# IC3Net/IC3Net

Hardware: AMD Instinct MI355X
Metric: env-steps/sec (agents x envs x steps), rollout hot path (higher is better)
Workload: dtype f32

## Files before the change

ic3net_amd/csrc/bptt_kernels.hip:

```cpp
#include <hip/hip_runtime.h>

#include <algorithm>
#include <cstddef>
#include <type_traits>
#include <vector>

#include "enc_bwd.hpp"
#include "ic3_common.hpp"
#include "ps_common.hpp"

extern "C" int ic3_lstm_gates_backward_given(const float* gates, float* xh, int ldx, const float* h_prev, const void* lstm_wp3_bwd,
                                             const float* c_prev, const float* dh, const float* dc, float* dgates, float* dc_prev,
                                             float* dbias_partials, int accumulate, float* dxh, const float* row_live,
                                             const float* row_keep, const float* dhead, const float* w_heads, int OT, int R, int H,
                                             ic3_stream stream);

namespace ic3 {

typedef float bp_f32x2 __attribute__((ext_vector_type(2)));
typedef float bp_f32x4 __attribute__((ext_vector_type(4)));
typedef float bp_f32x16 __attribute__((ext_vector_type(16)));

__device__ __forceinline__ __amdgpu_buffer_rsrc_t bp_rsrc(const void* base, long long bytes)
{
    const uint32_t n = bytes <= 0 ? 0u : (bytes > 0xffffffffll ? 0xffffffffu : (uint32_t)bytes);
    return __builtin_amdgcn_make_buffer_rsrc(const_cast<void*>(base), 0, n, 0x00020000);
}
__device__ __forceinline__ float bp_load1(__amdgpu_buffer_rsrc_t r, int voff, int soff = 0)
{
    return __builtin_bit_cast(float, __builtin_amdgcn_raw_buffer_load_b32(r, voff, soff, 0));
}
__device__ __forceinline__ bp_f32x4 bp_load4(__amdgpu_buffer_rsrc_t r, int voff, int soff = 0)
{
    return __builtin_bit_cast(bp_f32x4, __builtin_amdgcn_raw_buffer_load_b128(r, voff, soff, 0));
}
__device__ __forceinline__ void bp_store4(bp_f32x4 v, __amdgpu_buffer_rsrc_t r, int voff, int soff = 0)
{
    __builtin_amdgcn_raw_buffer_store_b128(__builtin_bit_cast(ps_u32x4, v), r, voff, soff, 0);
}
__device__ __forceinline__ void bp_mfma(bp_f32x16& acc, float x, float y)
{
    acc = __builtin_amdgcn_mfma_f32_32x32x2f32(x, y, acc, 0, 0, 0);
}
template <int N>
__device__ __forceinline__ void bp_zero(bp_f32x16* acc)
{
#pragma unroll
    for (int n = 0; n < N; ++n)
#pragma unroll
        for (int i = 0; i < 16; ++i) acc[n][i] = 0.0f;
}

struct KSlice {
    long long q0, nq;
    int nstages;
};
__device__ __forceinline__ KSlice bp_kslice(long long Q, int rows_per_wg, int KT)
{
    const long long q0 = (long long)blockIdx.x * rows_per_wg;
    long long nq = Q - q0;
    if (nq > rows_per_wg) nq = rows_per_wg;
    if (nq < 0) nq = 0;
    return KSlice{ q0, nq, (int)((nq + KT - 1) / KT) };
}

struct CommBwdArgs {
    const float* dxh;
    const float* h_prev;
    const int32_t* alive;
    const int32_t* gate;
    const float* cw;
    const float* out_scale;
    float* dh_out;
    float* dcw_part;
    int ldd, E, N, ept, tiles, mode_avg, accumulate;
};

template <int H>
__global__ __launch_bounds__(2 * H, (H <= 128) ? 3 : 1) void comm_bwd_kernel(const CommBwdArgs a)
{
    constexpr int NT = 2 * H, H4 = H / 4, LDA = H + 4, LDA4 = LDA / 4, MB = H / 32, PER = 64 * H4 / NT;
    IC3_DYNAMIC_LDS(float, smem);
    float* const Am = smem;
    bp_f32x4* const Am4 = reinterpret_cast<bp_f32x4*>(smem);
    float* const sg = smem + 64 * LDA;
    float* const sal = sg + 64;
    const int tid = threadIdx.x, lane = tid & 63, w = tid >> 6, li = lane & 31, lh = lane >> 5;
    const int col = 32 * w + li;
    const int N = a.N;
    bp_f32x16 acc2[MB];
    bp_zero<MB>(acc2);
    const __amdgpu_buffer_rsrc_t rcw = bp_rsrc(a.cw, (long long)H * H * 4);

    for (int tile = blockIdx.x; tile < a.tiles; tile += gridDim.x) {
        const int e0 = tile * a.ept;
        const int ne = (a.E - e0) < a.ept ? (a.E - e0) : a.ept;
        const int rows = ne * N;
        const long long r0 = (long long)e0 * N;
        const __amdgpu_buffer_rsrc_t rdi = bp_rsrc(a.dxh + r0 * a.ldd, ((long long)(rows - 1) * a.ldd + H) * 4);
        const __amdgpu_buffer_rsrc_t rdd = bp_rsrc(a.dxh + r0 * a.ldd + H, ((long long)(rows - 1) * a.ldd + H) * 4);
        const __amdgpu_buffer_rsrc_t rhp = bp_rsrc(a.h_prev + r0 * H, (long long)rows * H * 4);
        bp_f32x4 v[PER];
#pragma unroll
        for (int i = 0; i < PER; ++i) {
            const int idx = tid + i * NT, row = idx / H4, c4 = idx - row * H4;
            v[i] = bp_load4(rdi, (row * a.ldd + 4 * c4) * 4);
        }
        float mg = 0.f, mal = 0.f;
        if (tid < 64 && tid < rows) {
            mal = a.alive ? (float)a.alive[r0 + tid] : 1.0f;
            mg = mal * (a.gate ? (float)a.gate[r0 + tid] : 1.0f);
        }
        bp_f32x16 acc1[2];
#pragma unroll
        for (int rt = 0; rt < 2; ++rt)
#pragma unroll
            for (int reg = 0; reg < 16; ++reg)
                acc1[rt][reg] = bp_load1(rdd, (4 * lh * a.ldd + col) * 4, (32 * rt + (reg & 3) + 8 * (reg >> 2)) * a.ldd * 4);
#pragma unroll
        for (int i = 0; i < PER; ++i) Am4[(tid + i * NT) / H4 * LDA4 + (tid + i * NT) % H4] = v[i];
        if (tid < 64) {
            sg[tid] = mg;
            sal[tid] = mal;
        }
        float hpv[32];
#pragma unroll
        for (int s = 0; s < 32; ++s) hpv[s] = bp_load1(rhp, (lh * H + col) * 4, 2 * s * H * 4);
        __syncthreads();
        for (int item = tid; item < ne * H4; item += NT) {
            const int el = item / H4, c4 = item - el * H4;
            float na = 0.f;
            for (int j = 0; j < N; ++j) na += sal[el * N + j];
            const int n_alive = (int)na;
            const float scale = (a.mode_avg && n_alive > 1) ? 1.0f / (float)(n_alive - 1) : 1.0f;
            bp_f32x4 S = { 0.f, 0.f, 0.f, 0.f };
            for (int i = 0; i < N; ++i) S = mask_fma4(sg[el * N + i], Am4[(el * N + i) * LDA4 + c4], S);
            for (int j = 0; j < N; ++j) {
                const float m = sg[el * N + j];
                const bp_f32x4 x = Am4[(el * N + j) * LDA4 + c4];
                Am4[(el * N + j) * LDA4 + c4] = comm_out4(m, S, x, scale);
            }
        }
        __syncthreads();
        float wv[4], wn[4];
#pragma unroll
        for (int j = 0; j < 4; ++j) wv[j] = bp_load1(rcw, (4 * lh * H + col) * 4, j * H * 4);
#pragma unroll 2
        for (int kb = 0; kb < H / 8; ++kb) {
#pragma unroll
            for (int j = 0; j < 4; ++j) wn[j] = bp_load1(rcw, (4 * lh * H + col) * 4, (8 * (kb + 1) + j) * H * 4);
            const bp_f32x4 a0 = Am4[li * LDA4 + 2 * kb + lh];
            const bp_f32x4 a1 = Am4[(32 + li) * LDA4 + 2 * kb + lh];
#pragma unroll
            for (int j = 0; j < 4; ++j) {
                bp_mfma(acc1[0], a0[j], wv[j]);
                bp_mfma(acc1[1], a1[j], wv[j]);
            }
#pragma unroll
            for (int j = 0; j < 4; ++j) wv[j] = wn[j];
        }
        {
            const __amdgpu_buffer_rsrc_t rout = bp_rsrc(a.dh_out + r0 * H, (long long)rows * H * 4);
            const __amdgpu_buffer_rsrc_t rsc = bp_rsrc(a.out_scale ? a.out_scale + r0 : a.dh_out, a.out_scale ? (long long)rows * 4 : 0);
#pragma unroll
            for (int rt = 0; rt < 2; ++rt)
#pragma unroll
                for (int reg = 0; reg < 16; ++reg) {
                    const int lc = 32 * rt + (reg & 3) + 8 * (reg >> 2);
                    float o = acc1[rt][reg];
                    if (a.out_scale) o *= bp_load1(rsc, 4 * lh * 4, lc * 4);
                    __builtin_amdgcn_raw_buffer_store_b32(__builtin_bit_cast(int, o), rout, (4 * lh * H + col) * 4, lc * H * 4, 0);
                }
        }
#pragma unroll 4
        for (int s = 0; s < 32; ++s) {
#pragma unroll
            for (int mb = 0; mb < MB; ++mb) bp_mfma(acc2[mb], Am[(2 * s + lh) * LDA + 32 * mb + li], hpv[s]);
        }
        __syncthreads();
    }
    float* dst = a.dcw_part + (size_t)blockIdx.x * H * H;
#pragma unroll
    for (int mb = 0; mb < MB; ++mb)
#pragma unroll
        for (int reg = 0; reg < 16; ++reg) {
            const int k = 32 * mb + (reg & 3) + 8 * (reg >> 2) + 4 * lh;
            if (a.accumulate) dst[k * H + col] += acc2[mb][reg];
            else dst[k * H + col] = acc2[mb][reg];
        }
}

__global__ __launch_bounds__(256) void dh_copy_kernel(const float* __restrict__ dxh, int ldd, const float* __restrict__ out_scale,
                                                      float* __restrict__ dh_out, long long R, int H4)
{
    for (long long i = (long long)blockIdx.x * blockDim.x + threadIdx.x; i < R * H4; i += (long long)gridDim.x * blockDim.x) {
        const long long row = i / H4;
        const int c4 = (int)(i - row * H4);
        bp_f32x4 v = *reinterpret_cast<const bp_f32x4*>(dxh + row * ldd + 4 * H4 + 4 * c4);
        if (out_scale) v *= out_scale[row];
        reinterpret_cast<bp_f32x4*>(dh_out)[i] = v;
    }
}

struct WGradArgs {
    const float* inp;
    const float* h;
    const float* dg;
    const float* row_live;
    float* part;
    long long Q;
    int ldi, rows_per_wg;
};

template <int H>
__global__ __launch_bounds__(256, 2) void lstm_wgrad_kernel(const WGradArgs a)
{
    constexpr bool WIDE = H == 256;
    constexpr int HT = WIDE ? 128 : H;
    constexpr int KT = 16, XW = 2 * HT, DW = 128, MB = HT / 32, NB = 2, NT = 256;
    constexpr int X4R = XW / 4, D4R = DW / 4;
    constexpr int XPT = KT * X4R / NT, DPT = KT * D4R / NT;
    static_assert(XPT >= 1 && DPT == 2 && (NT % X4R) == 0, "staging split");
    IC3_DYNAMIC_LDS(float, smem);
    constexpr int SW = KT * (XW + DW);
    const int tid = threadIdx.x, lane = tid & 63, w = tid >> 6, li = lane & 31, lh = lane >> 5;
    const int wm = w & 1, wn = w >> 1;
    const int ny = blockIdx.y;
    const KSlice sl = bp_kslice(a.Q, a.rows_per_wg, KT);
    const long long q0 = sl.q0, nq = sl.nq;
    const int nstages = sl.nstages;
    const __amdgpu_buffer_rsrc_t ri = bp_rsrc(a.inp + q0 * a.ldi, nq > 0 ? ((nq - 1) * a.ldi + H) * 4 : 0);
    const __amdgpu_buffer_rsrc_t rh = bp_rsrc(a.h + q0 * H, nq * H * 4);
    const __amdgpu_buffer_rsrc_t rd = bp_rsrc(a.dg + q0 * 4 * H + ny * DW, nq > 0 ? ((nq - 1) * 4 * H + DW) * 4 : 0);
    const __amdgpu_buffer_rsrc_t rl = bp_rsrc(a.row_live ? a.row_live + q0 : a.h, a.row_live ? nq * 4 : 0);
    const int xrow = tid / X4R, xc4 = tid - xrow * X4R;
    const bool x_is_h = WIDE ? blockIdx.z != 0 : xc4 >= H / 4;
    const int xvoff = x_is_h ? (xrow * H + 4 * xc4 - (WIDE ? 0 : H)) * 4 : (xrow * a.ldi + 4 * xc4) * 4;
    const int xstep = (NT / X4R) * (x_is_h ? H : a.ldi) * 4;
    const int drow = tid / D4R, dc4 = tid - drow * D4R;
    const int dvoff = (drow * 4 * H + 4 * dc4) * 4;

    bp_f32x4 xr[XPT], dr[DPT];
    auto fetch = [&](int s) {
        const int qb = s * KT;
#pragma unroll
        for (int i = 0; i < XPT; ++i) {
            if (x_is_h) {
                xr[i] = bp_load4(rh, xvoff + i * xstep, qb * H * 4);
                if (a.row_live) xr[i] *= bp_load1(rl, (xrow + i * (NT / X4R)) * 4, qb * 4);
            } else {
                xr[i] = bp_load4(ri, xvoff + i * xstep, qb * a.ldi * 4);
            }
        }
#pragma unroll
        for (int i = 0; i < DPT; ++i) dr[i] = bp_load4(rd, dvoff + i * (NT / D4R) * 4 * H * 4, qb * 4 * H * 4);
    };
    auto stash = [&](int b) {
        bp_f32x4* X4 = reinterpret_cast<bp_f32x4*>(smem + b * SW);
        bp_f32x4* D4 = reinterpret_cast<bp_f32x4*>(smem + b * SW + KT * XW);
#pragma unroll
        for (int i = 0; i < XPT; ++i) X4[tid + i * NT] = xr[i];
#pragma unroll
        for (int i = 0; i < DPT; ++i) D4[tid + i * NT] = dr[i];
    };
    bp_f32x16 acc[MB][NB];
    bp_zero<MB * NB>(&acc[0][0]);
    if (nstages > 0) {
        fetch(0);
        stash(0);
    }
    __syncthreads();
    for (int s = 0; s < nstages; ++s) {
// ... 88 lines not shown
        for (int j = 0; j < 8; ++j) dv[j] = bp_load1(rd, doff, (qb + j) * 4 * H * 4);
    };
    auto stash = [&](int b) {
        ps_u32x4* f = frag + b * SQ;
        ps_u32x4 pl[3];
#pragma unroll
        for (int i = 0; i < NGX; ++i) {
            const int g = tid + i * NT, c = g % XW, kg = g / XW;
            ps_split_frag(ps_f32x4{ xv[i][0], xv[i][1], xv[i][2], xv[i][3] }, ps_f32x4{ xv[i][4], xv[i][5], xv[i][6], xv[i][7] }, pl);
#pragma unroll
            for (int p = 0; p < 3; ++p) f[(p * 2 + kg) * XW + c] = pl[p];
        }
        ps_split_frag(ps_f32x4{ dv[0], dv[1], dv[2], dv[3] }, ps_f32x4{ dv[4], dv[5], dv[6], dv[7] }, pl);
#pragma unroll
        for (int p = 0; p < 3; ++p) f[3 * 2 * XW + (p * 2 + dkg) * DW + dcol] = pl[p];
    };
    bp_f32x16 acc[MB][NB];
    bp_zero<MB * NB>(&acc[0][0]);
    fetch(0);
    stash(0);
    fetch(1);
    __syncthreads();
#pragma unroll 1
    for (int s = 0; s < nstages; ++s) {
        const ps_u32x4* fx = frag + (s & 1) * SQ;
        const ps_u32x4* fd = fx + 3 * 2 * XW;
        ps_u32x4 bf[3][NB];
#pragma unroll
        for (int p = 0; p < 3; ++p)
#pragma unroll
            for (int nb = 0; nb < NB; ++nb) bf[p][nb] = fd[(p * 2 + lh) * DW + 64 * wn + 32 * nb + li];
        stash((s + 1) & 1);
#pragma unroll
        for (int mb = 0; mb < MB; ++mb) {
            ps_u32x4 af[3];
#pragma unroll
            for (int p = 0; p < 3; ++p) af[p] = fx[(p * 2 + lh) * XW + wm * HT + 32 * mb + li];
#pragma unroll
            for (int pb = 0; pb < 3; ++pb)
#pragma unroll
                for (int nb = 0; nb < NB; ++nb)
#pragma unroll
                    for (int pa = 2; pa >= 0; --pa)
                        acc[mb][nb] = __builtin_amdgcn_mfma_f32_32x32x16_bf16(__builtin_bit_cast(wg_bf16x8, af[pa]),
                                                                              __builtin_bit_cast(wg_bf16x8, bf[pb][nb]), acc[mb][nb], 0, 0, 0);
        }
        fetch(s + 2);
        __syncthreads();
    }
    float* dst = a.part + (size_t)blockIdx.x * 2 * H * 4 * H;
    const int m0 = WIDE ? (int)blockIdx.z * XW : 0;
#pragma unroll
    for (int mb = 0; mb < MB; ++mb)
#pragma unroll
        for (int nb = 0; nb < NB; ++nb)
#pragma unroll
            for (int reg = 0; reg < 16; ++reg) {
                const int m = m0 + wm * HT + 32 * mb + (reg & 3) + 8 * (reg >> 2) + 4 * lh;
                dst[(size_t)m * 4 * H + DW * ny + 64 * wn + 32 * nb + li] = acc[mb][nb][reg];
            }
}

__global__ __launch_bounds__(256) void wgrad_reduce_kernel(const float* __restrict__ part, int nparts, int n, float* __restrict__ dW,
                                                           int accumulate)
{
    const int i = blockIdx.x * blockDim.x + threadIdx.x;
    if (i >= n) return;
    float s = 0.f;
    for (int p = 0; p < nparts; ++p) s += part[(size_t)p * n + i];
    dW[i] = accumulate ? dW[i] + s : s;
}

}

extern "C" int ic3_comm_backward_partials(int E, int N)
{
    if (E <= 0 || N <= 0 || N > 64) return 0;
    const int ept = 64 / N, tiles = (E + ept - 1) / ept;
    constexpr int cap = 512;
    const int rounds = (tiles + cap - 1) / cap;
    return (tiles + rounds - 1) / rounds;
}

extern "C" int ic3_comm_backward(const float* dxh, int ldd, const float* h_prev, const int32_t* alive, const int32_t* gate,
                                 const float* c_weight, const float* out_scale, float* dh_out,
                                 float* dcw_partials, int accumulate, int E, int N, int H, int mode_avg, int comm_zero,
                                 ic3_stream stream)
{
    using namespace ic3;
    if (!dxh || !dh_out || E <= 0 || N <= 0) return fail(-22, "ic3_comm_backward: null argument");
    if (ldd < 2 * H || (ldd & 3) || (H & 3)) return fail(-22, "ic3_comm_backward: ldd a multiple of 4, >= 2 * hid_size");
    hipStream_t s = (hipStream_t)stream;
    if (comm_zero) {
        const long long R = (long long)E * N, n4 = R * (H / 4);
        const int blocks = (int)std::min<long long>((n4 + 255) / 256, 4096);
        return launch_kernel(dh_copy_kernel, dim3(blocks), dim3(256), 0, s, dxh, ldd, out_scale, dh_out, R, H / 4);
    }
    if (!h_prev || !c_weight || !dcw_partials) return fail(-22, "ic3_comm_backward: null argument");
    if (H != 64 && H != 128 && H != 256) return fail(-38, "ic3_comm_backward: hid_size 64 / 128 / 256");
    if (N > 64) return fail(-38, "ic3_comm_backward: at most 64 agents per env");
    const int ept = 64 / N, tiles = (E + ept - 1) / ept;
    if ((long long)64 * ldd * 4 >= (1ll << 31)) return fail(-22, "ic3_comm_backward: row stride too large");
    const CommBwdArgs a{ dxh, h_prev, alive, gate, c_weight, out_scale, dh_out, dcw_partials, ldd, E, N, ept, tiles,
                         mode_avg, accumulate };
    const int grid = ic3_comm_backward_partials(E, N);
    const size_t lds = ((size_t)64 * (H + 4) + 128) * sizeof(float);
    const auto kernel = H == 256 ? comm_bwd_kernel<256> : H == 128 ? comm_bwd_kernel<128> : comm_bwd_kernel<64>;
    const int rc = launch_kernel(kernel, dim3(grid), dim3(2 * H), lds, s, a);
    return rc < 0 ? rc : grid;
}

struct WGradPlan {
    int ks;
    long long per;
    bool fits;
};
static WGradPlan wgrad_plan(long long Q, int ny, long long row_floats)
{
    int ks = 2 * ic3::device_cus() / ny;
    const long long most = (Q + 15) / 16;
    if (ks > most) ks = (int)most;
    if (ks < 1) ks = 1;
    const long long per = ((Q + ks - 1) / ks + 15) / 16 * 16;
    return WGradPlan{ ks, per, per * row_floats * 4 < (1ll << 31) };
}

static int wgrad_reduce(const float* scratch, int ks, int n, float* dW, int accumulate, hipStream_t s)
{
    const int rc = ic3::launch_kernel(ic3::wgrad_reduce_kernel, dim3((n + 255) / 256), dim3(256), 0, s, scratch, ks, n, dW, accumulate);
    return rc < 0 ? rc : ks;
}

static WGradPlan wgrad_plan_rounds(long long Q, int ny, long long row_floats)
{
    WGradPlan pl = wgrad_plan(Q, ny, row_floats);
    const long long most = (Q + 15) / 16;
    const int round = pl.ks;
    for (long long m = 2; !pl.fits && round * m <= most; ++m) {
        pl.ks = (int)(round * m);
        pl.per = ((Q + pl.ks - 1) / pl.ks + 15) / 16 * 16;
        pl.fits = pl.per * row_floats * 4 < (1ll << 31);
    }
    return pl;
}
static WGradPlan lstm_wgrad_plan(long long Q, int H, long long row_floats)
{
    return H == 256 ? wgrad_plan_rounds(Q, 16, row_floats) : wgrad_plan(Q, 4 * H / 128, row_floats);
}
static WGradPlan rnn_wgrad_plan(long long Q, int H, long long row_floats)
{
    return H == 256 ? wgrad_plan_rounds(Q, 4, row_floats) : wgrad_plan(Q, 1, row_floats);
}

static int lstm_weight_grad(const float* inp, int ldi, const float* h_prev, const float* dgates, const float* row_live, long long Q,
                            int H, float* dW, int accumulate, int split, float* scratch, ic3_stream stream)
{
    using namespace ic3;
    if (!inp || !h_prev || !dgates || !dW || !scratch || Q <= 0) return fail(-22, "ic3_lstm_weight_grad: null argument");
    if (ldi < H || (ldi & 3)) return fail(-22, "ic3_lstm_weight_grad: ldi a multiple of 4, >= hid_size");
    const WGradPlan pl = lstm_wgrad_plan(Q, H, std::max(ldi, 4 * H));
    if (!pl.fits) return fail(-22, "ic3_lstm_weight_grad: a K slice must stay below 2 GB per operand (32-bit buffer offsets)");
    const WGradArgs a{ inp, h_prev, dgates, row_live, scratch, Q, ldi, (int)pl.per };
    hipStream_t s = (hipStream_t)stream;
    const auto kernel = split ? (H == 256 ? lstm_wgrad_split_kernel<256> : H == 128 ? lstm_wgrad_split_kernel<128> : lstm_wgrad_split_kernel<64>)
                              : (H == 256 ? lstm_wgrad_kernel<256> : H == 128 ? lstm_wgrad_kernel<128> : lstm_wgrad_kernel<64>);
    const int HT = H == 256 ? 128 : H;
    const size_t lds = split ? (size_t)2 * 3 * 2 * (2 * HT + 128) * 16 : (size_t)2 * 16 * (2 * HT + 128) * sizeof(float);
    const dim3 grid = H == 256 ? dim3(pl.ks, 8, 2) : dim3(pl.ks, 4 * H / 128);
    if (const int rc = launch_kernel(kernel, grid, dim3(256), lds, s, a); rc < 0) return rc;
    return wgrad_reduce(scratch, pl.ks, 2 * H * 4 * H, dW, accumulate, s);
}

extern "C" size_t ic3_lstm_weight_grad_scratch_floats(long long Q, int H)
{
    if (Q <= 0 || (H != 64 && H != 128)) return 0;
    return (size_t)wgrad_plan(Q, 4 * H / 128, 0).ks * 2 * H * 4 * H;
}

extern "C" int ic3_lstm_weight_grad(const float* inp, int ldi, const float* h_prev, const float* dgates, const float* row_live,
                                    long long Q, int H, float* dW, int accumulate, int split, float* scratch, ic3_stream stream)
{
    if (H != 64 && H != 128) return ic3::fail(-38, "ic3_lstm_weight_grad: hid_size 64 / 128");
    return lstm_weight_grad(inp, ldi, h_prev, dgates, row_live, Q, H, dW, accumulate, split, scratch, stream);
}

extern "C" size_t ic3_lstm_weight_grad_wide_scratch_floats(long long Q, int H, int ldi)
{
    if (Q <= 0 || (H != 64 && H != 128 && H != 256)) return 0;
    return (size_t)lstm_wgrad_plan(Q, H, std::max(ldi, 4 * H)).ks * 2 * H * 4 * H;
}

extern "C" int ic3_lstm_weight_grad_wide(const float* inp, int ldi, const float* h_prev, const float* dgates, const float* row_live,
// ... 16 lines not shown
        const ic3_tj_cfg& c = env->tj;
        const int WW = env->dims.window * env->dims.window, hdr = c.vocab_type ? 4 : 2;
        pl = enc_bwd_plan(c.E, c.N, c.N, H, env->dims.grid_h * env->dims.grid_w, hdr + WW);
    }
    return pl.csplit ? 1 : 0;
}

namespace ic3 {
struct BpttSide {
    hipStream_t stream = nullptr;
    hipEvent_t fork = nullptr, join = nullptr;
    bool ready = false;
};
static BpttSide* bptt_side()
{
    static BpttSide side[65];
    int dev = 0;
    if (hipGetDevice(&dev) != hipSuccess || dev < -1 || dev >= 64) return nullptr;
    BpttSide& sd = side[dev + 1];
    if (!sd.ready) {
        if (!sd.stream && hipStreamCreateWithFlags(&sd.stream, hipStreamNonBlocking) != hipSuccess) return nullptr;
        if ((!sd.fork && hipEventCreateWithFlags(&sd.fork, hipEventDisableTiming) != hipSuccess) ||
            (!sd.join && hipEventCreateWithFlags(&sd.join, hipEventDisableTiming) != hipSuccess))
            return nullptr;
        sd.ready = true;
    }
    return &sd;
}

template <class B>
static int window_open(const char* fn, const char* sname, const ic3_env* env, const B* b, int (*supported)(const ic3_env*, int),
                       const char* needs, bool ot_enosys)
{
    const std::string f = std::string(fn) + ": ";
    if (!env || !b) return fail(-22, f + "null argument");
    if (b->struct_size != sizeof(B))
        return fail(-22, f + sname + " has " + std::to_string(b->struct_size) + " bytes, this library's has " +
                             std::to_string(sizeof(B)) + " (header / library version mismatch)");
    if (b->T <= 0 || b->E <= 0 || b->N <= 0 || b->E != env->dims.E || b->N != env->dims.N)
        return fail(-22, f + "T, E, N must be positive and E, N the handle's");
    if (!supported(env, b->H)) return fail(-38, f + needs);
    if (ot_enosys) {
        if (b->OT < 1) return fail(-22, f + "OT >= 1");
        if (b->OT > 16) return fail(-38, f + "at most 16 output columns");
    } else if (b->OT < 1 || b->OT > 16) {
        return fail(-22, f + "1 <= OT <= 16");
    }
    return 0;
}

static int encoder_tail(ic3_env* env, const int32_t* snaps, int64_t snap_words, int T, const float* g, int ldg, int64_t g_step,
                        int H, float* work, int enc_first, bool window, ic3_stream stream)
{
    if (window) return ic3_env_encode_backward_window(env, snaps, snap_words, T, g, ldg, g_step, H, work, enc_first, stream);
    for (int t = T - 1; t >= 0; --t) {
        const int rc = ic3_env_encode_backward_accumulate(env, snaps + (size_t)t * snap_words, g + (size_t)t * g_step, ldg, H, work,
                                                          enc_first, stream);
        if (rc < 0) return rc;
        enc_first = 0;
    }
    return 0;
}

struct BpttCell {
    float* gates;
    const float* c_prev;
    const float* h_prev;
    float* dh;
    float* dc;
    bool cut;
    float* dxh;
    float* dbias;
    const float* row_live;
    const float* row_keep;
    const float* dhead;
    const float* w_heads;
    int OT;
    const void* lstm_wp3_bwd;
    const int32_t* alive;
    const int32_t* gate;
    const float* c_weight;
    const float* out_scale;
    float* dcw;
    hipEvent_t ev0, ev1;
};
static int bptt_cell_backward(const char* fn, const BpttCell& q, int Ec, int N, int H, int mode_avg, int comm_zero, hipStream_t sc)
{
    ic3_stream scv = (ic3_stream)sc;
    if (q.ev0 && hipEventRecord(q.ev0, sc) != hipSuccess) return fail(-5, std::string(fn) + ": hipEventRecord of a gate event failed");
    int rc = ic3_lstm_gates_backward_given(q.gates, nullptr, 0, nullptr, q.lstm_wp3_bwd, q.c_prev, q.cut ? nullptr : q.dh,
                                           q.cut ? nullptr : q.dc, q.gates, q.dc, q.dbias, 1, q.dxh, q.row_live, q.row_keep, q.dhead,
                                           q.dhead ? q.w_heads : nullptr, q.OT, Ec * N, H, scv);
    if (rc < 0) return rc;
    if (q.ev1 && hipEventRecord(q.ev1, sc) != hipSuccess) return fail(-5, std::string(fn) + ": hipEventRecord of a gate event failed");
    return ic3_comm_backward(q.dxh, 2 * H, q.h_prev, q.alive, q.gate, q.c_weight, q.out_scale, q.dh, q.dcw, 1, Ec, N, H, mode_avg,
                             comm_zero, scv);
}
}

static int bptt_passes_backward(ic3_env* env, const ic3_bptt_passes* b, ic3_stream stream)
{
    using namespace ic3;
    if (const int rc = window_open("ic3_bptt_backward (ic3_bptt_passes)", "ic3_bptt_passes", env, b, ic3_bptt_backward_supported,
                                   "hid_size 64 / 128 / 256, <= 64 agents, a grid whose encoder backward runs in its partial-sums form",
                                   false);
        rc < 0)
        return rc;
    const int T = b->T, E = b->E, N = b->N, H = b->H, P = b->passes;
    if (P < 2) return fail(-22, "ic3_bptt_backward (ic3_bptt_passes): passes >= 2 (one pass: ic3_bptt_backward)");
    if (ic3_env_encode_backward_window_work(env, H) <= 0)
        return fail(-38, "ic3_bptt_backward (ic3_bptt_passes): needs a configuration with ic3_env_encode_backward_window (the ring form)");
    if (!b->gates || !b->hs || !b->cs || !b->dhead || !b->snaps || !b->lstm_wp3_bwd || !b->w_heads || !b->dh || !b->dc || !b->dxh ||
        !b->dbias_partials || !b->enc_work || b->t_first < 0)
        return fail(-22, "ic3_bptt_backward (ic3_bptt_passes): null argument");
    if (!b->comm_zero && (!b->c_weight || !b->dcw_partials)) return fail(-22, "ic3_bptt_backward (ic3_bptt_passes): the passes' C.weight and partials");
    const long long R = (long long)E * N;
    if (b->dxh_step < R * 2 * H) return fail(-22, "ic3_bptt_backward (ic3_bptt_passes): dxh_step >= E * N * 2 * hid_size (the ring form)");
    for (int i = 0; i < P; ++i) {
        if (!b->gates[i] || !b->hs[i] || !b->cs[i] || !b->dxh[i] || !b->dbias_partials[i] ||
            (!b->comm_zero && (!b->c_weight[i] || !b->dcw_partials[i])))
            return fail(-22, "ic3_bptt_backward (ic3_bptt_passes): null argument of pass " + std::to_string(i));
    }
    if (R * 4 * H * 4 >= (1ll << 32))
        return fail(-22, "ic3_bptt_backward (ic3_bptt_passes): rows * 4 * hid_size floats must stay below 4 GB (the gate launch's 32-bit buffer "
                         "offsets)");
    if (b->detach_gap > 0 && (b->row_keep || b->keep_before))
        return fail(-22, "ic3_bptt_backward (ic3_bptt_passes): detach_gap > 0 with row_keep / keep_before (a detached step has no dc for "
                         "row_keep to scale: lock-step windows carry detach_gap, collection-mode windows the row factors)");
    hipStream_t s = (hipStream_t)stream;
    for (int t = T - 1; t >= 0; --t) {
        const bool detached = b->detach_gap > 0 && (b->t_first + t + 1) % b->detach_gap == 0;
        const float* keep_here = b->row_keep ? b->row_keep + (size_t)t * R : nullptr;
        const float* keep_front = t > 0 ? (b->row_keep ? b->row_keep + (size_t)(t - 1) * R : nullptr) : b->keep_before;
        for (int i = P - 1; i >= 0; --i) {
            const bool last = i == P - 1;
            BpttCell q{};
            q.gates = b->gates[i] + (size_t)t * R * 4 * H;
            q.c_prev = b->cs[i] + (size_t)t * R * H;
            q.h_prev = b->hs[i] + (size_t)t * R * H;
            q.dh = b->dh;
            q.dc = b->dc;
            q.cut = detached && last;
            q.dxh = b->dxh[i] + (size_t)t * (size_t)b->dxh_step;
            q.dbias = b->dbias_partials[i];
            q.dhead = last ? b->dhead + (size_t)t * R * b->OT : nullptr;
            q.w_heads = b->w_heads;
            q.OT = b->OT;
            q.lstm_wp3_bwd = b->lstm_wp3_bwd;
            q.alive = (b->alive && b->alive[t]) ? b->alive[t] : nullptr;
            q.gate = (b->gate && b->gate[t]) ? b->gate[t] : nullptr;
            q.c_weight = b->comm_zero ? nullptr : b->c_weight[i];
            q.dcw = b->comm_zero ? nullptr : b->dcw_partials[i];
            q.row_keep = last ? keep_here : nullptr;
            q.out_scale = i == 0 ? keep_front : nullptr;
            if (const int rc = bptt_cell_backward("ic3_bptt_backward (ic3_bptt_passes)", q, E, N, H, b->mode_avg, b->comm_zero, s); rc < 0) return rc;
        }
    }
    for (int i = 0; i < P; ++i) {
        const int rc = ic3_env_encode_backward_window(env, b->snaps, b->snap_words, T, b->dxh[i], 2 * H, b->dxh_step, H, b->enc_work,
                                                      (i == 0 && b->enc_first) ? 1 : 0, stream);
        if (rc < 0) return rc;
    }
    return 0;
}

static int bptt_walk_backward(ic3_env* env, const ic3_bptt_walk* b, ic3_stream stream)
{
    using namespace ic3;
    const char* const fn = "ic3_bptt_backward (ic3_bptt_walk)";
    const std::string f = std::string(fn) + ": ";
    if (const int rc = window_open(fn, "ic3_bptt_walk", env, b, ic3_bptt_backward_supported,
                                   "hid_size 64 / 128 / 256, <= 64 agents, a grid whose encoder backward runs in its partial-sums form",
                                   false);
        rc < 0)
        return rc;
    if (!b->gates || !b->hs || !b->cs || !b->dhead || !b->snaps || !b->lstm_wp3_bwd || !b->w_heads || !b->dh || !b->dc || !b->dxh ||
        !b->dbias_partials || !b->enc_work)
        return fail(-22, f + "null argument");
    const long long R = (long long)b->E * b->N;
    if (b->dxh_step < R * 2 * b->H || ic3_env_encode_backward_window_work(env, b->H) <= 0)
        return fail(-22, f + "dxh_step >= E * N * 2 * hid_size, on a configuration with ic3_env_encode_backward_window (the walk needs "
                             "the ring)");
    if (b->detach_gap > 0 && b->row_keep)
        return fail(-22, f + "detach_gap > 0 with row_keep (a detached step has no dc for row_keep to scale: lock-step windows carry "
                             "detach_gap, collection-mode windows row_live / row_keep)");
    if (R >= (1ll << 31) || b->max_workgroups < 0) return fail(-22, f + "R < 2^31, max_workgroups >= 0");
    if (const int rc = lstm_gates_backward_walk(b, stream); rc < 0) return rc;
    return ic3_env_encode_backward_window(env, b->snaps, b->snap_words, b->T, b->dxh, 2 * b->H, b->dxh_step, b->H, b->enc_work,
                                          b->enc_first, stream);
}

extern "C" int ic3_bptt_first_chain_envs(int E, int N)
{
    if (E < 128 || N <= 0) return E;
    return (E / 2) & ~63;
}

extern "C" int ic3_bptt_backward(ic3_env* env, const ic3_bptt* b, ic3_stream stream)
{
    using namespace ic3;
    static_assert(offsetof(ic3_bptt_passes, magic) == offsetof(ic3_bptt, T), "the tag sits where ic3_bptt holds T");
    if (b && (uint32_t)b->T == IC3_BPTT_PASSES_MAGIC)
        return bptt_passes_backward(env, reinterpret_cast<const ic3_bptt_passes*>(b), stream);
    static_assert(offsetof(ic3_bptt_walk, magic) == offsetof(ic3_bptt, T), "the tag sits where ic3_bptt holds T");
    static_assert(sizeof(ic3_bptt_walk) != sizeof(ic3_bptt) && sizeof(ic3_bptt_walk) != sizeof(ic3_bptt_passes),
                  "the descriptors are told apart by their sizes too");
    if (b && (uint32_t)b->T == IC3_BPTT_WALK_MAGIC) return bptt_walk_backward(env, reinterpret_cast<const ic3_bptt_walk*>(b), stream);
    if (const int rc = window_open("ic3_bptt_backward", "ic3_bptt", env, b, ic3_bptt_backward_supported,
                                   "hid_size 64 / 128 / 256, <= 64 agents, a grid whose encoder backward runs in its partial-sums form",
                                   false);
        rc < 0)
        return rc;
    const int T = b->T, E = b->E, N = b->N, H = b->H;
    if (!b->gates || !b->hs || !b->cs || !b->dhead || !b->snaps || !b->lstm_wp3_bwd || !b->w_heads || !b->dh || !b->dc || !b->dxh ||
        !b->dbias_partials || !b->enc_work)
        return fail(-22, "ic3_bptt_backward: null argument");
    if (!b->comm_zero && (!b->c_weight || !b->dcw_partials)) return fail(-22, "ic3_bptt_backward: C.weight and its partials");
    if (b->dxh_step && (b->dxh_step < (long long)E * N * 2 * H || ic3_env_encode_backward_window_work(env, H) <= 0))
        return fail(-22, "ic3_bptt_backward: dxh_step >= E * N * 2 * hid_size, on a configuration with ic3_env_encode_backward_window");
    if (b->detach_gap > 0 && b->row_keep)
        return fail(-22, "ic3_bptt_backward: detach_gap > 0 with row_keep (a detached step has no dc for row_keep to scale: lock-step "
                         "windows carry detach_gap, collection-mode windows row_live / row_keep)");
    const long long R = (long long)E * N;
    hipStream_t s = (hipStream_t)stream;
    const int E1 = (b->two_chains && b->dxh_step) ? ic3_bptt_first_chain_envs(E, N) : E;
    const int nch = E1 < E ? 2 : 1;
    if ((long long)std::max(E1, E - E1) * N * 4 * H * 4 >= (1ll << 32))
        return fail(-22, "ic3_bptt_backward: a chain's rows * 4 * hid_size floats must stay below 4 GB (the gate launch's 32-bit buffer "
                         "offsets)");
    BpttSide* side = nch == 2 ? bptt_side() : nullptr;
    if (nch == 2 && !side) return fail(-12, "ic3_bptt_backward: no second stream");
    if (nch == 2) {
        IC3_HIP(hipEventRecord(side->fork, s));
        IC3_HIP(hipStreamWaitEvent(side->stream, side->fork, 0));
    }
    auto join = [&](int rc) {
        if (nch == 2 && (hipEventRecord(side->join, side->stream) != hipSuccess || hipStreamWaitEvent(s, side->join, 0) != hipSuccess) &&
            rc >= 0)
            return fail(-5, "ic3_bptt_backward: joining the second stream failed");
        return rc;
    };
    int enc_first = b->enc_first;
    for (int t = T - 1; t >= 0; --t) {
        for (int ch = 0; ch < nch; ++ch) {
            const int e0 = ch ? E1 : 0, Ec = ch ? E - E1 : E1;
            const size_t r0 = (size_t)e0 * N;
            hipStream_t sc = ch ? side->stream : s;
            const bool detached = b->detach_gap > 0 && (t + 1) % b->detach_gap == 0;
            BpttCell q{};
            q.gates = b->gates + ((size_t)t * R + r0) * 4 * H;
            q.c_prev = b->cs + ((size_t)t * R + r0) * H;
            q.h_prev = b->hs + ((size_t)t * R + r0) * H;
            q.dh = b->dh + r0 * H;
            q.dc = b->dc + r0 * H;
            q.cut = detached;
            q.dxh = b->dxh + (size_t)t * (size_t)b->dxh_step + r0 * 2 * H;
            q.dbias = b->dbias_partials + (r0 / 64) * 4 * H;
            q.row_live = b->row_live ? b->row_live + (size_t)t * R + r0 : nullptr;
            q.row_keep = b->row_keep ? b->row_keep + (size_t)t * R + r0 : nullptr;
            q.dhead = b->dhead + ((size_t)t * R + r0) * b->OT;
            q.w_heads = b->w_heads;
            q.OT = b->OT;
            q.lstm_wp3_bwd = b->lstm_wp3_bwd;
            q.alive = (b->alive && b->alive[t]) ? b->alive[t] + r0 : nullptr;
            q.gate = (b->gate && b->gate[t]) ? b->gate[t] + r0 : nullptr;
            q.c_weight = b->c_weight;
            q.out_scale = (b->row_keep && t > 0) ? b->row_keep + (size_t)(t - 1) * R + r0 : nullptr;
            q.dcw = b->dcw_partials;
            if (q.dcw && ch) q.dcw += (size_t)ic3_comm_backward_partials(E1, N) * H * H;
            if (b->gate_events && ch == 0) {
                q.ev0 = (hipEvent_t)b->gate_events[2 * t];
                q.ev1 = (hipEvent_t)b->gate_events[2 * t + 1];
            }
            const int rc = bptt_cell_backward("ic3_bptt_backward", q, Ec, N, H, b->mode_avg, b->comm_zero, sc);
            if (rc < 0) return join(rc);
        }
        if (b->dxh_step) continue;
        int rc = ic3_env_encode_backward_accumulate(env, b->snaps + (size_t)t * b->snap_words, b->dxh, 2 * H, H, b->enc_work,
                                                    enc_first, stream);
        if (rc < 0) return join(rc);
        enc_first = 0;
    }
    if (const int rc = join(0); rc < 0) return rc;
    if (b->dxh_step)
        return ic3_env_encode_backward_window(env, b->snaps, b->snap_words, T, b->dxh, 2 * H, b->dxh_step, H, b->enc_work, enc_first,
                                              stream);
    return 0;
}

namespace ic3 {

template <int H>
struct TanhTile {
    static constexpr int NT = 4 * H, H4 = H / 4, LDA = H + 4, LDA4 = LDA / 4, CB = H / 32, RPP = NT / H4, PER = 64 / RPP;
    static_assert(RPP * PER == 64 && NT / 64 == 2 * CB, "tile split");
    static constexpr bool RESIDENT = H <= 128;
    static constexpr int DZ_AT = RESIDENT ? H * H : 0, WH_AT = DZ_AT + 64 * LDA, SD_AT = WH_AT + 16 * H;
    static constexpr size_t LDS_BYTES = (size_t)(SD_AT + 64 * 16) * sizeof(float);
    float* const smem;
    const bp_f32x4* const Bf4;
    float* const Dz;
    bp_f32x4* const Dz4;
    float* const Wh;
    float* const Sd;
    const int tid, li, lh;
    const int cb, rb;
    const int c4, rg;

    __device__ __forceinline__ explicit TanhTile(float* lds)
        : smem(lds), Bf4(reinterpret_cast<const bp_f32x4*>(lds)), Dz(lds + DZ_AT), Dz4(reinterpret_cast<bp_f32x4*>(lds + DZ_AT)),
          Wh(lds + WH_AT), Sd(lds + SD_AT), tid(threadIdx.x), li(threadIdx.x & 31), lh((threadIdx.x & 63) >> 5),
          cb((threadIdx.x >> 6) % CB), rb((threadIdx.x >> 6) / CB), c4(threadIdx.x % H4), rg(threadIdx.x / H4)
    {
    }
    __device__ __forceinline__ void stage_weights(const float* a2, const float* w_heads, int OT) const
    {
        if constexpr (RESIDENT) {
            for (int i = tid; i < H * H; i += NT) {
                const int k = i / H, col = i - k * H;
                smem[(((k >> 3) * 2 + ((k >> 2) & 1)) * H + col) * 4 + (k & 3)] = a2[i];
            }
        }
        for (int i = tid; i < OT * H; i += NT) Wh[i] = w_heads[i];
    }
    __device__ __forceinline__ bp_f32x4 heads_share(bp_f32x4 v, int row, int OT) const
    {
        const bp_f32x4* const Wh4 = reinterpret_cast<const bp_f32x4*>(Wh);
        for (int o = 0; o < OT; ++o) v += Sd[row * OT + o] * Wh4[o * H4 + c4];
        return v;
    }
    __device__ __forceinline__ bp_f32x16 product(const float* a2) const
    {
        bp_f32x16 acc;
        bp_zero<1>(&acc);
        if constexpr (RESIDENT) {
#pragma unroll 4
            for (int kb = 0; kb < H / 8; ++kb) {
                const bp_f32x4 a4 = Dz4[(32 * rb + li) * LDA4 + 2 * kb + lh];
                const bp_f32x4 b4 = Bf4[(2 * kb + lh) * H + 32 * cb + li];
#pragma unroll
                for (int j = 0; j < 4; ++j) bp_mfma(acc, a4[j], b4[j]);
            }
        } else {
            const __amdgpu_buffer_rsrc_t ra = bp_rsrc(a2, (long long)H * H * 4);
            const int voff = (4 * lh * H + 32 * cb + li) * 4;
            float bv[8], bn[8];
#pragma unroll
            for (int j = 0; j < 8; ++j) bv[j] = bp_load1(ra, voff, (8 * (j >> 2) + (j & 3)) * H * 4);
#pragma unroll 2
            for (int kb = 0; kb < H / 8; kb += 2) {
#pragma unroll
                for (int j = 0; j < 8; ++j) bn[j] = bp_load1(ra, voff, (8 * (kb + 2 + (j >> 2)) + (j & 3)) * H * 4);
                const bp_f32x4 a0 = Dz4[(32 * rb + li) * LDA4 + 2 * kb + lh];
                const bp_f32x4 a1 = Dz4[(32 * rb + li) * LDA4 + 2 * kb + 2 + lh];
#pragma unroll
                for (int j = 0; j < 4; ++j) bp_mfma(acc, a0[j], bv[j]);
#pragma unroll
                for (int j = 0; j < 4; ++j) bp_mfma(acc, a1[j], bv[4 + j]);
#pragma unroll
                for (int j = 0; j < 8; ++j) bv[j] = bn[j];
            }
        }
        return acc;
    }
    __device__ __forceinline__ void column_sums(bp_f32x4 bsum, float* db_part, int accumulate) const
    {
// ... 866 lines not shown
```

Measured before the change: 275.2 million.

## Defer comm weight-gradient accumulation out of the BPTT chain into windowed launches

Splits the comm backward kernel into modes. The per-step chain launch (mode 1) now only computes dh through the comm weights and skips the dC weight-gradient MFMA accumulation and the h_prev loads. The dC gradient is computed after the reverse-time loop by a windowed kernel (mode 2) that covers up to 32 timesteps per launch, software-prefetches the next tile's inputs, and accumulates into the existing partial buffers. This shortens the serial critical path of the BPTT chain at the cost of re-reading dxh and hs in a separate pass. It also adds an environment knob to restore the in-chain behaviour.

```diff
diff --git a/ic3net_amd/csrc/bptt_kernels.hip b/ic3net_amd/csrc/bptt_kernels.hip
--- a/ic3net_amd/csrc/bptt_kernels.hip
+++ b/ic3net_amd/csrc/bptt_kernels.hip
@@ -2,6 +2,7 @@
 
 #include <algorithm>
 #include <cstddef>
+#include <cstdlib>
 #include <type_traits>
 #include <vector>
 
@@ -76,8 +77,20 @@
     int ldd, E, N, ept, tiles, mode_avg, accumulate;
 };
 
-template <int H>
-__global__ __launch_bounds__(2 * H, (H <= 128) ? 3 : 1) void comm_bwd_kernel(const CommBwdArgs a)
+constexpr int COMM_WIN_STEPS = 32;
+struct CommWinArgs {
+    const float* dxh;
+    const float* h_prev;
+    float* dcw_part;
+    long long dxh_step, h_step;
+    int ldd, E, N, ept, tiles, mode_avg, nsteps;
+    const int32_t* alive[COMM_WIN_STEPS];
+    const int32_t* gate[COMM_WIN_STEPS];
+};
+
+template <int H, int MODE>
+__global__ __launch_bounds__(2 * H, MODE == 1 ? 4 : MODE == 2 ? ((H <= 128) ? 2 : 1) : ((H <= 128) ? 3 : 1))
+void comm_bwd_kernel(const std::conditional_t<MODE == 2, CommWinArgs, CommBwdArgs> a)
 {
     constexpr int NT = 2 * H, H4 = H / 4, LDA = H + 4, LDA4 = LDA / 4, MB = H / 32, PER = 64 * H4 / NT;
     IC3_DYNAMIC_LDS(float, smem);
@@ -88,45 +101,102 @@
     const int tid = threadIdx.x, lane = tid & 63, w = tid >> 6, li = lane & 31, lh = lane >> 5;
     const int col = 32 * w + li;
     const int N = a.N;
-    bp_f32x16 acc2[MB];
-    bp_zero<MB>(acc2);
-    const __amdgpu_buffer_rsrc_t rcw = bp_rsrc(a.cw, (long long)H * H * 4);
-
-    for (int tile = blockIdx.x; tile < a.tiles; tile += gridDim.x) {
-        const int e0 = tile * a.ept;
+    bp_f32x16 acc2[MODE == 1 ? 1 : MB];
+    if constexpr (MODE != 1) bp_zero<MB>(acc2);
+    [[maybe_unused]] __amdgpu_buffer_rsrc_t rcw;
+    if constexpr (MODE != 2) rcw = bp_rsrc(a.cw, (long long)H * H * 4);
+    [[maybe_unused]] bp_f32x4 vn[MODE == 2 ? PER : 1];
+    constexpr bool HP_AHEAD = H <= 128;
+    [[maybe_unused]] float mgn = 0.f, maln = 0.f, hpn[(MODE == 2 && HP_AHEAD) ? 32 : 1];
+    [[maybe_unused]] auto fetch = [&](int item) {
+        if constexpr (MODE == 2) {
+            const int t = item / a.tiles, e0 = (item - t * a.tiles) * a.ept;
+            const int rows = ((a.E - e0) < a.ept ? (a.E - e0) : a.ept) * N;
+            const long long r0 = (long long)e0 * N;
+            const __amdgpu_buffer_rsrc_t rdi = bp_rsrc(a.dxh + (long long)t * a.dxh_step + r0 * a.ldd, ((long long)(rows - 1) * a.ldd + H) * 4);
+            [[maybe_unused]] const __amdgpu_buffer_rsrc_t rhp = bp_rsrc(a.h_prev + (long long)t * a.h_step + r0 * H, (long long)rows * H * 4);
+#pragma unroll
+            for (int i = 0; i < PER; ++i) {
+                const int idx = tid + i * NT, row = idx / H4, c4 = idx - row * H4;
+                vn[i] = bp_load4(rdi, (row * a.ldd + 4 * c4) * 4);
+            }
+            mgn = 0.f, maln = 0.f;
+            if (tid < 64 && tid < rows) {
+                const int32_t* const al = a.alive[t];
+                const int32_t* const gt = a.gate[t];
+                maln = al ? (float)al[r0 + tid] : 1.0f;
+                mgn = maln * (gt ? (float)gt[r0 + tid] : 1.0f);
+            }
+            if constexpr (HP_AHEAD) {
+#pragma unroll
+                for (int s = 0; s < 32; ++s) hpn[s] = bp_load1(rhp, (lh * H + col) * 4, 2 * s * H * 4);
+            }
+        }
+    };
+    int items;
+    if constexpr (MODE == 2) {
+        items = a.nsteps * a.tiles;
+        if ((int)blockIdx.x < items) fetch(blockIdx.x);
+    } else {
+        items = a.tiles;
+    }
+
+    for (int tile = blockIdx.x; tile < items; tile += gridDim.x) {
+        int e0;
+        if constexpr (MODE == 2) e0 = tile % a.tiles * a.ept;
+        else e0 = tile * a.ept;
         const int ne = (a.E - e0) < a.ept ? (a.E - e0) : a.ept;
         const int rows = ne * N;
         const long long r0 = (long long)e0 * N;
-        const __amdgpu_buffer_rsrc_t rdi = bp_rsrc(a.dxh + r0 * a.ldd, ((long long)(rows - 1) * a.ldd + H) * 4);
-        const __amdgpu_buffer_rsrc_t rdd = bp_rsrc(a.dxh + r0 * a.ldd + H, ((long long)(rows - 1) * a.ldd + H) * 4);
-        const __amdgpu_buffer_rsrc_t rhp = bp_rsrc(a.h_prev + r0 * H, (long long)rows * H * 4);
+        [[maybe_unused]] __amdgpu_buffer_rsrc_t rhp;
         bp_f32x4 v[PER];
-#pragma unroll
-        for (int i = 0; i < PER; ++i) {
-            const int idx = tid + i * NT, row = idx / H4, c4 = idx - row * H4;
-            v[i] = bp_load4(rdi, (row * a.ldd + 4 * c4) * 4);
-        }
         float mg = 0.f, mal = 0.f;
-        if (tid < 64 && tid < rows) {
-            mal = a.alive ? (float)a.alive[r0 + tid] : 1.0f;
-            mg = mal * (a.gate ? (float)a.gate[r0 + tid] : 1.0f);
-        }
-        bp_f32x16 acc1[2];
-#pragma unroll
-        for (int rt = 0; rt < 2; ++rt)
-#pragma unroll
-            for (int reg = 0; reg < 16; ++reg)
-                acc1[rt][reg] = bp_load1(rdd, (4 * lh * a.ldd + col) * 4, (32 * rt + (reg & 3) + 8 * (reg >> 2)) * a.ldd * 4);
+        [[maybe_unused]] bp_f32x16 acc1[2];
+        if constexpr (MODE != 2) {
+            const __amdgpu_buffer_rsrc_t rdi = bp_rsrc(a.dxh + r0 * a.ldd, ((long long)(rows - 1) * a.ldd + H) * 4);
+            const __amdgpu_buffer_rsrc_t rdd = bp_rsrc(a.dxh + r0 * a.ldd + H, ((long long)(rows - 1) * a.ldd + H) * 4);
+            if constexpr (MODE == 0) rhp = bp_rsrc(a.h_prev + r0 * H, (long long)rows * H * 4);
+#pragma unroll
+            for (int i = 0; i < PER; ++i) {
+                const int idx = tid + i * NT, row = idx / H4, c4 = idx - row * H4;
+                v[i] = bp_load4(rdi, (row * a.ldd + 4 * c4) * 4);
+            }
+            if (tid < 64 && tid < rows) {
+                mal = a.alive ? (float)a.alive[r0 + tid] : 1.0f;
+                mg = mal * (a.gate ? (float)a.gate[r0 + tid] : 1.0f);
+            }
+#pragma unroll
+            for (int rt = 0; rt < 2; ++rt)
+#pragma unroll
+                for (int reg = 0; reg < 16; ++reg)
+                    acc1[rt][reg] = bp_load1(rdd, (4 * lh * a.ldd + col) * 4, (32 * rt + (reg & 3) + 8 * (reg >> 2)) * a.ldd * 4);
+        } else {
+#pragma unroll
+            for (int i = 0; i < PER; ++i) v[i] = vn[i];
+            mg = mgn, mal = maln;
+        }
 #pragma unroll
         for (int i = 0; i < PER; ++i) Am4[(tid + i * NT) / H4 * LDA4 + (tid + i * NT) % H4] = v[i];
         if (tid < 64) {
             sg[tid] = mg;
             sal[tid] = mal;
         }
-        float hpv[32];
-#pragma unroll
-        for (int s = 0; s < 32; ++s) hpv[s] = bp_load1(rhp, (lh * H + col) * 4, 2 * s * H * 4);
-        __syncthreads();
+        [[maybe_unused]] float hpv[MODE == 1 ? 1 : 32];
+        if constexpr (MODE == 0) {
+#pragma unroll
+            for (int s = 0; s < 32; ++s) hpv[s] = bp_load1(rhp, (lh * H + col) * 4, 2 * s * H * 4);
+        } else if constexpr (MODE == 2 && HP_AHEAD) {
+#pragma unroll
+            for (int s = 0; s < 32; ++s) hpv[s] = hpn[s];
+        } else if constexpr (MODE == 2) {
+            rhp = bp_rsrc(a.h_prev + (long long)(tile / a.tiles) * a.h_step + r0 * H, (long long)rows * H * 4);
+#pragma unroll
+            for (int s = 0; s < 32; ++s) hpv[s] = bp_load1(rhp, (lh * H + col) * 4, 2 * s * H * 4);
+        }
+        __syncthreads();
+        if constexpr (MODE == 2) {
+            if (tile + (int)gridDim.x < items) fetch(tile + gridDim.x);
+        }
         for (int item = tid; item < ne * H4; item += NT) {
             const int el = item / H4, c4 = item - el * H4;
             float na = 0.f;
@@ -142,6 +212,7 @@
             }
         }
         __syncthreads();
+        if constexpr (MODE != 2) {
         float wv[4], wn[4];
 #pragma unroll
         for (int j = 0; j < 4; ++j) wv[j] = bp_load1(rcw, (4 * lh * H + col) * 4, j * H * 4);
@@ -172,22 +243,29 @@
                     __builtin_amdgcn_raw_buffer_store_b32(__builtin_bit_cast(int, o), rout, (4 * lh * H + col) * 4, lc * H * 4, 0);
                 }
         }
+        }
+        if constexpr (MODE != 1) {
 #pragma unroll 4
         for (int s = 0; s < 32; ++s) {
 #pragma unroll
             for (int mb = 0; mb < MB; ++mb) bp_mfma(acc2[mb], Am[(2 * s + lh) * LDA + 32 * mb + li], hpv[s]);
         }
-        __syncthreads();
-    }
+        }
+        __syncthreads();
+    }
+    if constexpr (MODE != 1) {
     float* dst = a.dcw_part + (size_t)blockIdx.x * H * H;
+    bool accumulate = true;
+    if constexpr (MODE == 0) accumulate = a.accumulate;
 #pragma unroll
     for (int mb = 0; mb < MB; ++mb)
 #pragma unroll
         for (int reg = 0; reg < 16; ++reg) {
             const int k = 32 * mb + (reg & 3) + 8 * (reg >> 2) + 4 * lh;
-            if (a.accumulate) dst[k * H + col] += acc2[mb][reg];
+            if (accumulate) dst[k * H + col] += acc2[mb][reg];
             else dst[k * H + col] = acc2[mb][reg];
         }
+    }
 }
 
 __global__ __launch_bounds__(256) void dh_copy_kernel(const float* __restrict__ dxh, int ldd, const float* __restrict__ out_scale,
@@ -442,12 +520,11 @@
     return (tiles + rounds - 1) / rounds;
 }
 
-extern "C" int ic3_comm_backward(const float* dxh, int ldd, const float* h_prev, const int32_t* alive, const int32_t* gate,
-                                 const float* c_weight, const float* out_scale, float* dh_out,
-                                 float* dcw_partials, int accumulate, int E, int N, int H, int mode_avg, int comm_zero,
-                                 ic3_stream stream)
-{
-    using namespace ic3;
+namespace ic3 {
+static int comm_backward(const float* dxh, int ldd, const float* h_prev, const int32_t* alive, const int32_t* gate,
+                         const float* c_weight, const float* out_scale, float* dh_out, float* dcw_partials, int accumulate, int E, int N,
+                         int H, int mode_avg, int comm_zero, bool chain, ic3_stream stream)
+{
     if (!dxh || !dh_out || E <= 0 || N <= 0) return fail(-22, "ic3_comm_backward: null argument");
     if (ldd < 2 * H || (ldd & 3) || (H & 3)) return fail(-22, "ic3_comm_backward: ldd a multiple of 4, >= 2 * hid_size");
     hipStream_t s = (hipStream_t)stream;
@@ -456,18 +533,62 @@
         const int blocks = (int)std::min<long long>((n4 + 255) / 256, 4096);
         return launch_kernel(dh_copy_kernel, dim3(blocks), dim3(256), 0, s, dxh, ldd, out_scale, dh_out, R, H / 4);
     }
-    if (!h_prev || !c_weight || !dcw_partials) return fail(-22, "ic3_comm_backward: null argument");
+    if (!c_weight || (!chain && (!h_prev || !dcw_partials))) return fail(-22, "ic3_comm_backward: null argument");
     if (H != 64 && H != 128 && H != 256) return fail(-38, "ic3_comm_backward: hid_size 64 / 128 / 256");
     if (N > 64) return fail(-38, "ic3_comm_backward: at most 64 agents per env");
     const int ept = 64 / N, tiles = (E + ept - 1) / ept;
     if ((long long)64 * ldd * 4 >= (1ll << 31)) return fail(-22, "ic3_comm_backward: row stride too large");
     const CommBwdArgs a{ dxh, h_prev, alive, gate, c_weight, out_scale, dh_out, dcw_partials, ldd, E, N, ept, tiles,
                          mode_avg, accumulate };
+    const size_t lds = ((size_t)64 * (H + 4) + 128) * sizeof(float);
+    if (chain) {
+        const int grid = tiles;
+        const auto kernel = H == 256 ? comm_bwd_kernel<256, 1> : H == 128 ? comm_bwd_kernel<128, 1> : comm_bwd_kernel<64, 1>;
+        const int rc = launch_kernel(kernel, dim3(grid), dim3(2 * H), lds, s, a);
+        return rc < 0 ? rc : 0;
+    }
     const int grid = ic3_comm_backward_partials(E, N);
-    const size_t lds = ((size_t)64 * (H + 4) + 128) * sizeof(float);
-    const auto kernel = H == 256 ? comm_bwd_kernel<256> : H == 128 ? comm_bwd_kernel<128> : comm_bwd_kernel<64>;
+    const auto kernel = H == 256 ? comm_bwd_kernel<256, 0> : H == 128 ? comm_bwd_kernel<128, 0> : comm_bwd_kernel<64, 0>;
     const int rc = launch_kernel(kernel, dim3(grid), dim3(2 * H), lds, s, a);
     return rc < 0 ? rc : grid;
+}
+
+static int comm_dcw_window(const float* dxh, long long dxh_step, const float* hs, const int32_t* const* alive,
+                           const int32_t* const* gate, float* dcw_partials, int slots, int T, int E, int N, int H, int mode_avg,
+                           hipStream_t s)
+{
+    const int ept = 64 / N, tiles = (E + ept - 1) / ept;
+    if ((long long)tiles * COMM_WIN_STEPS >= (1ll << 30)) return fail(-22, "ic3_bptt_backward: too many row tiles for the dC launch");
+    const size_t lds = ((size_t)64 * (H + 4) + 128) * sizeof(float);
+    const long long R = (long long)E * N;
+    const int resident = H == 256 ? 256 : 512;
+    for (int t0 = 0; t0 < T; t0 += COMM_WIN_STEPS) {
+        CommWinArgs a{};
+        a.nsteps = std::min(COMM_WIN_STEPS, T - t0);
+        a.dxh = dxh + (size_t)t0 * (size_t)dxh_step;
+        a.h_prev = hs + (size_t)t0 * (size_t)R * H;
+        a.dcw_part = dcw_partials;
+        a.dxh_step = dxh_step, a.h_step = R * H;
+        a.ldd = 2 * H, a.E = E, a.N = N, a.ept = ept, a.tiles = tiles, a.mode_avg = mode_avg;
+        for (int i = 0; i < a.nsteps; ++i) {
+            a.alive[i] = (alive && alive[t0 + i]) ? alive[t0 + i] : nullptr;
+            a.gate[i] = (gate && gate[t0 + i]) ? gate[t0 + i] : nullptr;
+        }
+        const int grid = std::max(1, std::min(std::min(slots, resident), a.nsteps * tiles));
+        const auto kernel = H == 256 ? comm_bwd_kernel<256, 2> : H == 128 ? comm_bwd_kernel<128, 2> : comm_bwd_kernel<64, 2>;
+        if (const int rc = launch_kernel(kernel, dim3(grid), dim3(2 * H), lds, s, a); rc < 0) return rc;
+    }
+    return 0;
+}
+}
+
+extern "C" int ic3_comm_backward(const float* dxh, int ldd, const float* h_prev, const int32_t* alive, const int32_t* gate,
+                                 const float* c_weight, const float* out_scale, float* dh_out,
+                                 float* dcw_partials, int accumulate, int E, int N, int H, int mode_avg, int comm_zero,
+                                 ic3_stream stream)
+{
+    return ic3::comm_backward(dxh, ldd, h_prev, alive, gate, c_weight, out_scale, dh_out, dcw_partials, accumulate, E, N, H, mode_avg,
+                              comm_zero, false, stream);
 }
 
 struct WGradPlan {
@@ -650,6 +771,7 @@
     const float* c_weight;
     const float* out_scale;
     float* dcw;
+    bool dcw_deferred;
     hipEvent_t ev0, ev1;
 };
 static int bptt_cell_backward(const char* fn, const BpttCell& q, int Ec, int N, int H, int mode_avg, int comm_zero, hipStream_t sc)
@@ -661,8 +783,8 @@
                                            q.dhead ? q.w_heads : nullptr, q.OT, Ec * N, H, scv);
     if (rc < 0) return rc;
     if (q.ev1 && hipEventRecord(q.ev1, sc) != hipSuccess) return fail(-5, std::string(fn) + ": hipEventRecord of a gate event failed");
-    return ic3_comm_backward(q.dxh, 2 * H, q.h_prev, q.alive, q.gate, q.c_weight, q.out_scale, q.dh, q.dcw, 1, Ec, N, H, mode_avg,
-                             comm_zero, scv);
+    return comm_backward(q.dxh, 2 * H, q.h_prev, q.alive, q.gate, q.c_weight, q.out_scale, q.dh, q.dcw, 1, Ec, N, H, mode_avg,
+                         comm_zero, q.dcw_deferred, scv);
 }
 }
 
@@ -793,6 +915,10 @@
     hipStream_t s = (hipStream_t)stream;
     const int E1 = (b->two_chains && b->dxh_step) ? ic3_bptt_first_chain_envs(E, N) : E;
     const int nch = E1 < E ? 2 : 1;
+    constexpr bool DCW_IN_CHAIN_DEFAULT = false;
+    const char* const knob = getenv("IC3_BPTT_DCW_IN_CHAIN");
+    const bool in_chain = (knob && (knob[0] == '0' || knob[0] == '1') && !knob[1]) ? knob[0] == '1' : DCW_IN_CHAIN_DEFAULT;
+    const bool dcw_deferred = b->dxh_step && !b->comm_zero && !in_chain;
     if ((long long)std::max(E1, E - E1) * N * 4 * H * 4 >= (1ll << 32))
         return fail(-22, "ic3_bptt_backward: a chain's rows * 4 * hid_size floats must stay below 4 GB (the gate launch's 32-bit buffer "
                          "offsets)");
@@ -836,6 +962,7 @@
             q.out_scale = (b->row_keep && t > 0) ? b->row_keep + (size_t)(t - 1) * R + r0 : nullptr;
             q.dcw = b->dcw_partials;
             if (q.dcw && ch) q.dcw += (size_t)ic3_comm_backward_partials(E1, N) * H * H;
+            q.dcw_deferred = dcw_deferred;
             if (b->gate_events && ch == 0) {
                 q.ev0 = (hipEvent_t)b->gate_events[2 * t];
                 q.ev1 = (hipEvent_t)b->gate_events[2 * t + 1];
@@ -850,6 +977,13 @@
         enc_first = 0;
     }
     if (const int rc = join(0); rc < 0) return rc;
+    if (dcw_deferred) {
+        const int slots = ic3_comm_backward_partials(E1, N) + (nch == 2 ? ic3_comm_backward_partials(E - E1, N) : 0);
+        if (const int rc = comm_dcw_window(b->dxh, b->dxh_step, b->hs, b->alive, b->gate, b->dcw_partials, slots, T, E, N, H,
+                                           b->mode_avg, s);
+            rc < 0)
+            return rc;
+    }
     if (b->dxh_step)
         return ic3_env_encode_backward_window(env, b->snaps, b->snap_words, T, b->dxh, 2 * H, b->dxh_step, H, b->enc_work, enc_first,
                                               stream);
```

Result: no change. 273.3 million (-0.7%).
